# mit-han-lab/qserve

Hardware: AMD Instinct MI355X
Metric: decode tokens/sec/GPU Llama-3-8B W4A8KV4 bs=64 (higher is better)
Workload: dtype int8xint4->int32 (MFMA) + fp16; 1 GPU; Llama-3-8B W4A8 per-channel KV4 decode step, bs=64, context 1024->+512 (BASELINE.json configs[1]); global_batch=64, context_start=1030, parallelism=tp1, hipgraph=True, layers=32, launches_per_layer=8

## Files before the change

qserve_amd/csrc/attention.hip:

```cpp
#include "common.h"
#include "kv_quant.h"

namespace {

constexpr int TPB = 256;
constexpr int PAGE_TOK = 64;
constexpr int DH = 128;

__device__ __forceinline__ void nib8_to_h2(u32 x, h2 (&o)[4]) {
    const u32 t = x >> 8;
    u32 w0 = (x & 0x000F000Fu) | 0x64006400u;
    u32 w1 = (x & 0x00F000F0u) | 0x64006400u;
    u32 w2 = (t & 0x000F000Fu) | 0x64006400u;
    u32 w3 = (t & 0x00F000F0u) | 0x64006400u;
    const h2 k1024 = {(_Float16)1024.f, (_Float16)1024.f};
    const h2 k16 = {(_Float16)0.0625f, (_Float16)0.0625f};
    const h2 km64 = {(_Float16)-64.f, (_Float16)-64.f};
    o[0] = __builtin_bit_cast(h2, w0) - k1024;
    o[1] = __builtin_elementwise_fma(__builtin_bit_cast(h2, w1), k16, km64);
    o[2] = __builtin_bit_cast(h2, w2) - k1024;
    o[3] = __builtin_elementwise_fma(__builtin_bit_cast(h2, w3), k16, km64);
}

template <bool INT4>
// ... 546 lines not shown
        case 2: QS_LAUNCH_G(2); break;
        case 3: QS_LAUNCH_G(3); break;
        case 4: QS_LAUNCH_G(4); break;
        case 5: QS_LAUNCH_G(5); break;
        case 6: QS_LAUNCH_G(6); break;
        case 7: QS_LAUNCH_G(7); break;
        case 8: QS_LAUNCH_G(8); break;
        default:
            qs_set_error("single_query_attention: num_heads/num_kv_heads = %d not in 1..8", G);
            return QS_ENOSUP;
    }
#undef QS_LAUNCH_G
    return qs_launch_status("single_query_attention");
}

}

const float2* qs_rope_table(float base, int max_pos, hipStream_t st, int* len_out);
int qs_launch_decode_mfma(int G, dim3 grid, hipStream_t st, const _Float16* q, const _Float16* k, const _Float16* v,
                          const int64_t* kvp, const int* len, _Float16* out, int H, int Hkv, int64_t qs, int64_t kvs,
                          int mb, int timestep, float base, int max_pos, int nsplit, int kflags, int exp_flags,
                          const QsAttnQuant* quant, bool* fused);
int qs_launch_decode_mfma8(int G, dim3 grid, hipStream_t st, const _Float16* q, const _Float16* k, const _Float16* v,
                           const int64_t* kvp, const int* len, _Float16* out, int H, int Hkv, int64_t qs, int64_t kvs,
                           int mb, int timestep, float base, int max_pos, int nsplit);
namespace {

qs_flag g_attn_variant = 0;

int qs_attn_choose_splits(int blocks, int pages, int kv8, int fused_quant) {
    if (blocks >= 512 || pages < 4) return 1;
    const long F = kv8 ? 5000 : 4000, t_cu = kv8 ? 450 : 340, t_hbm_ps = kv8 ? 2540 : 1330;
    long best = -1;
    int best_n = 1;
    for (int n = 1; n <= 8; ++n) {
        if (n > 1 && pages / n < 2) break;
        const long rounds = ((long)blocks * n + 255) / 256;
        const long per_cu = rounds * pages * t_cu / n, chip = (long)blocks * pages * t_hbm_ps / 1000;
        const long cost = rounds * F + (per_cu > chip ? per_cu : chip) + (n > 1 ? 2500 + 300 * n + (fused_quant ? 3500 : 0) : 0);
        if (best < 0 || cost < best) best = cost, best_n = n;
    }
    return best_n;
}
struct AttnPlan {
    int family, nsplit, waves, kflags, exp_flags;
};
AttnPlan plan_attention(int batch, int H, int Hkv, int max_blocks, int timestep, bool int4, bool fused_quant, int variant) {
    const int G = H / Hkv;
    if (G < 1 || G > 8) {
        qs_set_error("single_query_attention: num_heads/num_kv_heads = %d not in 1..8", G);
        return {0};
    }
    if (variant == 1 || max_blocks > 192) return {3, 1, TPB / 64};
    int force_split = variant >= 100 ? variant - 100 : 0, exp_flags = 0;
    if (int4 && force_split >= 100) {
        exp_flags = force_split - 100;
        force_split = 0;
    }
    const int blocks = Hkv * batch;
    const int pages_max = (timestep + PAGE_TOK - 1) / PAGE_TOK;
    const int nsplit = force_split > 0 ? force_split : qs_attn_choose_splits(blocks, pages_max, int4 ? 0 : 1, int4 && fused_quant && H * DH <= 4096);
    if (int4) return {1, nsplit, QS_ATTN_WAVES_KV4, variant == 5 ? 2 : variant == 7 ? 1024 : 0, exp_flags};
    return {2, nsplit, QS_ATTN_WAVES_KV8};
}

int single_query_attention(const void* q, const void* k, const void* v, const int64_t* kv_pointers,
                           const int32_t* length_per_sample, void* out, int batch, int num_heads, int num_kv_heads,
                           int head_dim, int64_t q_stride0, int64_t kv_stride0, int max_blocks, int memory_max_seqlen,
                           int tokens_per_block, int size_per_token, int timestep, int rotary_embedding_dim,
                           float rotary_base, int neox_rotary_style, int int4_kv_cache, int kv_cache_with_zeros,
                           qs_stream_t stream, const QsAttnQuant* quant, bool* fused) {
    QS_REQUIRE(q && k && v && kv_pointers && out, "single_query_attention: null pointer");
    QS_REQUIRE(batch >= 0 && num_heads > 0 && num_kv_heads > 0 && num_heads % num_kv_heads == 0,
               "single_query_attention: bad head counts H=%d Hkv=%d", num_heads, num_kv_heads);
    (void)neox_rotary_style;
    if (head_dim != 128 || rotary_embedding_dim != 128 || tokens_per_block != 64 || !kv_cache_with_zeros) {
        qs_set_error("single_query_attention: only head_dim=128, rotary_dim=128, tokens_per_block=64 and "
                     "zero-point KV caches are supported (the variants the reference instantiates)");
        return QS_ENOSUP;
    }
    const int dhb = int4_kv_cache ? 64 : 128;
    QS_REQUIRE(size_per_token == num_kv_heads * dhb, "single_query_attention: size_per_token=%d, expected %d",
               size_per_token, num_kv_heads * dhb);
    QS_REQUIRE(max_blocks > 0 && memory_max_seqlen > 0, "single_query_attention: bad max_blocks / memory_max_seqlen");
    QS_REQUIRE(q_stride0 % 8 == 0 && kv_stride0 % 8 == 0 && q_stride0 >= (int64_t)num_heads * 128 && kv_stride0 >= (int64_t)num_kv_heads * 128,
               "single_query_attention: token strides must hold the token's heads and keep 16-byte alignment");
    QS_REQUIRE(((reinterpret_cast<uintptr_t>(q) | reinterpret_cast<uintptr_t>(k) | reinterpret_cast<uintptr_t>(v) |
                 reinterpret_cast<uintptr_t>(out)) & 15) == 0,
               "single_query_attention: q, k, v and out must be 16-byte aligned");
    if (batch == 0) return QS_OK;
    const AttnPlan plan = plan_attention(batch, num_heads, num_kv_heads, max_blocks, timestep, int4_kv_cache, quant != nullptr,
                                         g_attn_variant);
    if (!plan.family) return QS_ENOSUP;
    dim3 grid(num_kv_heads, batch);
    const int G = num_heads / num_kv_heads;
    hipStream_t st = (hipStream_t)stream;
    const _Float16 *q16 = (const _Float16*)q, *k16 = (const _Float16*)k, *v16 = (const _Float16*)v;
    if (plan.family == 1)
        return qs_launch_decode_mfma(G, grid, st, q16, k16, v16, kv_pointers, length_per_sample, (_Float16*)out, num_heads,
                                     num_kv_heads, q_stride0, kv_stride0, max_blocks, timestep, rotary_base, memory_max_seqlen,
                                     plan.nsplit, plan.kflags, plan.exp_flags, quant, fused);
    if (plan.family == 2)
        return qs_launch_decode_mfma8(G, grid, st, q16, k16, v16, kv_pointers, length_per_sample, (_Float16*)out, num_heads,
                                      num_kv_heads, q_stride0, kv_stride0, max_blocks, timestep, rotary_base, memory_max_seqlen,
                                      plan.nsplit);
    if (int4_kv_cache)
        return launch_decode<true>(G, grid, st, q16, k16, v16, kv_pointers, length_per_sample, (_Float16*)out, num_heads,
                                   num_kv_heads, q_stride0, kv_stride0, max_blocks, timestep, rotary_base);
    return launch_decode<false>(G, grid, st, q16, k16, v16, kv_pointers, length_per_sample, (_Float16*)out, num_heads,
                                num_kv_heads, q_stride0, kv_stride0, max_blocks, timestep, rotary_base);
}

}

extern "C" void qs_set_attention_variant(int variant) { g_attn_variant = variant; }
// ... 157 lines not shown
```

qserve_amd/csrc/attention_mfma.hip:

```cpp
#include "common.h"
#include "kv_quant.h"
#include <mutex>

namespace {

constexpr int PAGE_TOK = 64;
constexpr int DH = 128;
constexpr int DHB = 64;
constexpr int UT = 32;
constexpr int USB = UT * DHB;
constexpr int NW = QS_ATTN_WAVES_KV4;
constexpr int NWT = NW;
constexpr int QS_ATTNQ_CAP = 4096;
constexpr int QS_ATTNQ_ROW = 4096;
constexpr int SVC = NW - 1;
#ifndef QS_SEQ
#define QS_SEQ(x) asm volatile("" : "+v"(x))
#endif
constexpr int MAXP = 192;

typedef __attribute__((address_space(1))) uint8_t* g_u8;
typedef __attribute__((address_space(1))) uint16_t* g_u16;
__device__ __forceinline__ void wave_quant_store4(_Float16 v0, _Float16 v1, uint8_t* dst_, __half* scale_p_,
                                                  __half* zero_p_, int lane) {
    g_u8 dst = (g_u8)dst_;
    g_u16 scale_p = (g_u16)reinterpret_cast<uint16_t*>(scale_p_), zero_p = (g_u16)reinterpret_cast<uint16_t*>(zero_p_);
    const float mx = wave_max_dpp(fmaxf((float)v0, (float)v1));
    const float mn = wave_min_dpp(fminf((float)v0, (float)v1));
    const QParams p = make_qparams<true>(mn, mx);
    const unsigned u0 = quant_u8(v0, p), u1 = quant_u8(v1, p);
    dst[lane] = (uint8_t)((u0 & 0xFu) | (u1 << 4));
    if (lane == 0) {
        *scale_p = __builtin_bit_cast(uint16_t, p.scale);
        *zero_p = __builtin_bit_cast(uint16_t, p.zero);
    }
}

__device__ __forceinline__ u32 and_or(u32 x, u32 m, u32 c) {
    return (x & m) | c;
}

typedef __attribute__((address_space(3))) const uint8_t* lds_u8;

template <int G, int EXP = 0>
__global__ __launch_bounds__(NWT * 64, 4) void decode_attention_mfma_kernel(
    const _Float16* __restrict__ q, const _Float16* __restrict__ k, const _Float16* __restrict__ v,
    const int64_t* __restrict__ kv_pointers, const int* __restrict__ lengths, _Float16* __restrict__ out,
    int num_heads, int num_kv_heads, int64_t q_stride0, int64_t kv_stride0, int max_blocks, int timestep,
    float rope_base, const float2* __restrict__ rope_tab, int rope_tab_len, int nsplit, float* __restrict__ ws,
    int8_t* __restrict__ qout, __half* __restrict__ qscale, __half* __restrict__ qrowsum, unsigned* __restrict__ qcounters,
    int kflags) {
    __shared__ __attribute__((aligned(16))) uint8_t s_kv[2 * NW * 2 * USB];
    __shared__ __attribute__((aligned(16))) _Float16 s_meta[NW][2][4][UT];
    __shared__ __attribute__((aligned(16))) _Float16 s_q[G][DH];
    __shared__ __attribute__((aligned(16))) _Float16 s_qp[16][DH];
    __shared__ __attribute__((aligned(16))) _Float16 s_knew[DH];
    __shared__ __attribute__((aligned(16))) _Float16 s_vnew[DH];
    __shared__ float s_cur[16];
    __shared__ float2 s_qc[16];
    __shared__ float s_m[NW][G], s_l[NW][G];
    __shared__ int s_flag;

    const int tid = threadIdx.x, lane = tid & 63;
    const int wave = __builtin_amdgcn_readfirstlane(tid >> 6);
    const int hkv = blockIdx.x, b = blockIdx.y;
    __shared__ unsigned long long s_stamps[(EXP & 32) ? NWT * 16 : 1];
    auto stamp = [&](int i) {
        if constexpr (EXP & 32) {
            const unsigned long long t = __builtin_amdgcn_s_memtime();
            if (lane == 0) s_stamps[wave * 16 + i] = t;
        }
    };
    if constexpr (EXP & 32) {
        if (lane < 16) s_stamps[wave * 16 + lane] = 0;
    }
    stamp(0);
    if (!(kflags & 2)) {
        const u32 fa = (u32)(uintptr_t)(__attribute__((address_space(3))) void*)(&s_flag);
        if (tid == SVC * 64) asm volatile("ds_write_b32 %0, %1" ::"v"(fa), "v"(0));
        asm volatile("s_waitcnt lgkmcnt(0)\n\ts_barrier");
    }
    const _Float16* qb = q + (size_t)b * q_stride0 + (size_t)hkv * G * DH;
    const _Float16* kb = k + (size_t)b * kv_stride0 + (size_t)hkv * DH;
    const _Float16* vb = v + (size_t)b * kv_stride0 + (size_t)hkv * DH;
    auto uni_ptr = [](const void* x) -> uint64_t {
        return ((uint64_t)(u32)__builtin_amdgcn_readfirstlane((u32)((uint64_t)(uintptr_t)x >> 32)) << 32) |
               (uint64_t)(u32)__builtin_amdgcn_readfirstlane((u32)(uint64_t)(uintptr_t)x);
    };
    const uint64_t qb_s = uni_ptr(qb), kb_s = uni_ptr(kb), vb_s = uni_ptr(vb);
    const int64_t* ktab = kv_pointers + (size_t)b * 2 * max_blocks;
    const int64_t* vtab = ktab + max_blocks;
    const bool spec = (nsplit == 1 || blockIdx.z == 0);
    if (wave == SVC) {
        asm volatile("s_setprio 3");
        if constexpr (!(EXP & 4)) {
            const u32 lane4 = (u32)lane * 4u;
            auto glds4 = [&](uint64_t sb, const _Float16* dst) {
                const u32 ld = __builtin_amdgcn_readfirstlane((u32)(uintptr_t)(__attribute__((address_space(3))) const void*)dst);
                asm volatile("s_mov_b32 m0, %2\n\ts_nop 4\n\tglobal_load_lds_dword %0, %1" ::"v"(lane4), "s"(sb), "s"(ld) : "memory");
            };
#pragma unroll
            for (int h = 0; h < G; ++h) glds4(qb_s + (uint64_t)(h * DH * 2), &s_q[h][0]);
            glds4(kb_s, &s_knew[0]);
            glds4(vb_s, &s_vnew[0]);
        }
        stamp(5);
    }
    int64_t kpage0, vpage0, kpage7, vpage7;
    int len_raw, gen_raw;
    {
        const int p0 = (wave >> 1) < max_blocks ? (wave >> 1) : 0, p7 = ((wave + NW - 1) >> 1) < max_blocks ? ((wave + NW - 1) >> 1) : 0;
        const uint64_t a0 = uni_ptr(ktab + p0), a1 = uni_ptr(vtab + p0), a2 = uni_ptr(ktab + p7), a3 = uni_ptr(vtab + p7);
        const uint64_t a4 = uni_ptr(lengths ? (const void*)(lengths + b) : (const void*)ktab);
        const uint64_t a5 = uni_ptr(qcounters ? (const void*)(qcounters + b) : (const void*)ktab);
        asm volatile("s_load_dwordx2 %0, %6, 0x0\n\ts_load_dwordx2 %1, %7, 0x0\n\ts_load_dwordx2 %2, %8, 0x0\n\t"
                     "s_load_dwordx2 %3, %9, 0x0\n\ts_load_dword %4, %10, 0x0\n\ts_load_dword %5, %11, 0x0\n\ts_waitcnt lgkmcnt(0)"
                     : "=&s"(kpage0), "=&s"(vpage0), "=&s"(kpage7), "=&s"(vpage7), "=&s"(len_raw), "=&s"(gen_raw)
                     : "s"(a0), "s"(a1), "s"(a2), "s"(a3), "s"(a4), "s"(a5)
                     : "memory");
    }
    const int tl = lengths ? len_raw - 1 : timestep;
    if (tl < 0) return;
    stamp(1);
    const float inv_sqrt = 0.08838834764831845f;
    const float qk_scale = inv_sqrt * 1.4426950408889634f;
    constexpr int GP = G <= 4 ? 4 : 8;
    const int li = lane & 15, tg = lane >> 4;
// ... 338 lines not shown
            for (int j = 0; j < NS; ++j) {
                const float pe = __builtin_amdgcn_exp2f(sc[j] - m_new);
                l_part += pe;
                float ps = (float)(_Float16)(pe * vsf[j]);
                float pz = ps * vzf[j];
                if (!full && tok0 + j >= valid) {
                    ps = 0.f;
                    pz = 0.f;
                }
                corr += pz;
                psum += ps;
                pp[j] = ps;
            }
            if constexpr (GP == 4) {
                const int pk = (int)pack_h2(pp[0], pp[1]);
                pbv[0] = (u32)pk;
                pbv[1] = (u32)__builtin_amdgcn_update_dpp(0, pk, 0x104, 0xF, 0xF, true);
                pbv[2] = (u32)__builtin_amdgcn_update_dpp(0, pk, 0x108, 0xF, 0xF, true);
                pbv[3] = (u32)__builtin_amdgcn_update_dpp(0, pk, 0x10C, 0xF, 0xF, true);
            } else {
                const int pk0 = (int)pack_h2(pp[0], pp[1]), pk1 = (int)pack_h2(pp[2], pp[3]);
                pbv[0] = (u32)pk0;
                pbv[1] = (u32)pk1;
                pbv[2] = (u32)__builtin_amdgcn_update_dpp(0, pk0, 0x108, 0xF, 0xF, true);
                pbv[3] = (u32)__builtin_amdgcn_update_dpp(0, pk1, 0x108, 0xF, 0xF, true);
            }
        }
        {
            const h8 pB = __builtin_bit_cast(h8, (v4u){pbv[0], pbv[1], pbv[2], pbv[3]});
            u32 raw[8];
#pragma unroll
            for (int jj = 0; jj < 8; ++jj) {
                raw[jj] = *(const __attribute__((address_space(3))) u32*)(vl + (16 * (jj >> 2) + (jj & 3)) * DHB);
            }
#pragma unroll
            for (int bb = 0; bb < 4; ++bb) {
                u32 lo[4], hi[4];
#pragma unroll
                for (int pq = 0; pq < 4; ++pq) {
                    const u32 W = __builtin_amdgcn_perm(raw[2 * pq + 1], raw[2 * pq], 0x0c000c00u | bb | ((4u + bb) << 16));
                    lo[pq] = and_or(W, c_lo, c_magic);
                    hi[pq] = and_or(W, c_hi, c_magic);
                }
                const h8 a_lo = __builtin_bit_cast(h8, (v4u){lo[0], lo[1], lo[2], lo[3]});
                const h8 a_hi = __builtin_bit_cast(h8, (v4u){hi[0], hi[1], hi[2], hi[3]});
                acc[2 * bb] = __builtin_amdgcn_mfma_f32_16x16x32_f16(a_lo, pB, acc[2 * bb], 0, 0, 0);
                acc[2 * bb + 1] = __builtin_amdgcn_mfma_f32_16x16x32_f16(a_hi, pB, acc[2 * bb + 1], 0, 0, 0);
            }
        }
        asm volatile("s_waitcnt lgkmcnt(0) ; QS_LOOP_END" ::: "memory");
        if (it < 2) stamp(6 + 2 * it);
        if (has2) dma_b(vpage_next, u2 & 1, slot, valid2);
    }

    const u32 lid2 = fresh_lane_id();
    const int li2 = lid2 & 15, tg2 = lid2 >> 4, tid2 = wave * 64 + (int)lid2;
    if constexpr (GP == 4) {
        l_part += xor_lane(l_part, lid2, 4);
        corr += xor_lane(corr, lid2, 4);
        psum += xor_lane(psum, lid2, 4);
    }
    l_part += xor_lane(l_part, lid2, 8);
    corr += xor_lane(corr, lid2, 8);
    psum += xor_lane(psum, lid2, 8);
    l_part += xor_lane(l_part, lid2, 16);
    l_part += xor_lane(l_part, lid2, 32);
    corr += xor_lane(corr, lid2, 16);
    corr += xor_lane(corr, lid2, 32);
    psum += xor_lane(psum, lid2, 16);
    psum += xor_lane(psum, lid2, 32);
    if constexpr (!(EXP & 4)) {
        if (wave == SVC && !svc_free) new_token_work();
    }
    asm volatile("s_waitcnt vmcnt(0)" ::: "memory");
    stamp(12);
    __syncthreads();
    stamp(13);
    constexpr int OS = DH + 4;
    float (*s_o)[G][OS] = reinterpret_cast<float (*)[G][OS]>(&s_kv[0]);
    static_assert(sizeof(float) * NW * G * OS <= sizeof(s_kv), "merge area must fit the page buffers");
    if (li2 < G) {
#pragma unroll
        for (int e = 0; e < 8; ++e)
#pragma unroll
            for (int r = 0; r < 4; ++r)
                s_o[wave][li2][8 * (4 * tg2 + r) + e] = ((e & 1) ? acc[e][r] * 0.0625f : acc[e][r]) - (corr + ((e & 1) ? 64.f : 1024.f) * psum);
        if (tg2 == 0) {
            s_m[wave][li2] = m_run;
            s_l[wave][li2] = l_part;
        }
    }
    __syncthreads();
    stamp(14);
    for (int o = tid2; o < G * DH; o += NWT * 64) {
        const int h = o / DH, d = o % DH;
        float M = z == 0 ? s_cur[h] : -3.0e38f;
#pragma unroll
        for (int w = 0; w < NW; ++w) M = fmaxf(M, s_m[w][h]);
        const float pc = z == 0 ? __builtin_amdgcn_exp2f(s_cur[h] - M) : 0.f;
        float num = pc * (float)((EXP & 4) ? vb[d] : s_vnew[d]), den = pc;
#pragma unroll
        for (int w = 0; w < NW; ++w) {
            const float f = __builtin_amdgcn_exp2f(s_m[w][h] - M);
            num += f * s_o[w][h][d];
            den += f * s_l[w][h];
        }
        if (nsplit == 1) {
            const _Float16 res = (_Float16)(num / (den + 1.e-6f));
            if (qout) reinterpret_cast<_Float16*>(&s_meta[0][0][0])[o] = res;
            else out[((size_t)b * num_heads + (size_t)hkv * G + h) * DH + d] = res;
        } else {
            float* pw = ws + ((((size_t)b * num_kv_heads + hkv) * nsplit + z) * G + h) * (DH + 2);
            pw[d] = num;
            if (d == 0) {
                pw[DH] = M * 0.6931471805599453f;
                pw[DH + 1] = den;
            }
        }
    }
    if (nsplit == 1 && qout) {
        __syncthreads();
        const int hidden = num_heads * DH;
        const unsigned tag = (unsigned)gen_raw + 1u;
        if (tid2 < G * 16) {
            const v4u x = reinterpret_cast<const v4u*>(&s_meta[0][0][0])[tid2];
            *reinterpret_cast<v4u*>(out + ((size_t)b * num_heads + (size_t)hkv * G) * DH + tid2 * 8) = x;
        }
        v2u* const xrow = reinterpret_cast<v2u*>(qcounters + QS_ATTNQ_CAP) + (size_t)b * (QS_ATTNQ_ROW / 2);
        const int own_lo = (num_kv_heads - 1) * G * DH;
        if ((G == 4 || G == 8) && !(kflags & 1024)) {
            float* const sm = reinterpret_cast<float*>(&s_kv[0]);
            v4u* const gran = reinterpret_cast<v4u*>(xrow);
            if (wave == 0) {
                const int ln = (int)lid2;
                float amax = 0.f, s0 = 0.f, s1 = 0.f;
                {
                    const h8 vv = __builtin_bit_cast(h8, reinterpret_cast<const v4u*>(&s_meta[0][0][0])[ln]);
#pragma unroll
                    for (int j = 0; j < 8; ++j) {
                        const float f = (float)vv[j];
                        s0 += f;
                        QS_SEQ(s0);
                        amax = fmaxf(amax, fabsf(f));
                    }
                }
                if (G == 8) {
                    const h8 vv = __builtin_bit_cast(h8, reinterpret_cast<const v4u*>(&s_meta[0][0][0])[64 + ln]);
#pragma unroll
                    for (int j = 0; j < 8; ++j) {
                        const float f = (float)vv[j];
                        s1 += f;
                        QS_SEQ(s1);
                        amax = fmaxf(amax, fabsf(f));
                    }
                }
                amax = wave_max(amax);
                s0 = wave_sum(s0);
                if (G == 8) s1 = wave_sum(s1);
                v4u mine = {__builtin_bit_cast(u32, amax), __builtin_bit_cast(u32, s0), __builtin_bit_cast(u32, s1), tag};
                if (ln == 0 && !((kflags & 64) && b == 0 && hkv == 0) && !(kflags & 512)) {
                    v4u* const dst = gran + hkv;
                    asm volatile("global_store_dwordx4 %0, %1, off sc0 sc1" ::"v"(dst), "v"(mine) : "memory");
                }
                const __amdgpu_buffer_rsrc_t grs = __builtin_amdgcn_make_buffer_rsrc(gran, 0, num_kv_heads * 16, 0x00020000);
                const bool peer = ln < num_kv_heads && ln != hkv;
                const u32 goff = ln < num_kv_heads ? (u32)ln * 16u : 0xFFFFFF00u;
                const int spin_cap = (kflags & 256) ? 1 : (kflags & 64) ? 4096 : QS_SPIN_CAP;
                int polls = 0;
                v4u g;
                for (;;) {
                    g = __builtin_amdgcn_raw_buffer_load_b128(grs, goff, 0, 17);
                    if (!__builtin_amdgcn_ballot_w64(peer && g.w != tag)) break;
                    if (++polls >= spin_cap) {
                        if (ln == 0 && !(kflags & 256))
                            atomicOr(qcounters + QS_ATTNQ_CAP + (size_t)QS_ATTNQ_CAP * QS_ATTNQ_ROW, QS_ERR_ATTN_HANDOVER);
                        break;
                    }
                    __builtin_amdgcn_s_sleep(1);
                }
                if (ln == hkv) g = mine;
                const u32 gx = g.x, gy = g.y, gz = g.z;
                float am = ln < num_kv_heads ? __builtin_bit_cast(float, gx) : 0.f;
                am = wave_max(am);
                float bs;
                if (G == 4) {
                    bs = ln < num_kv_heads ? __builtin_bit_cast(float, gy) : -0.0f;
                } else {
                    const int src = (ln >> 1) < num_kv_heads ? (ln >> 1) : 0;
                    const int yv = __builtin_amdgcn_ds_bpermute(4 * src, (int)gy), zv = __builtin_amdgcn_ds_bpermute(4 * src, (int)gz);
                    bs = (ln >> 1) < num_kv_heads ? __builtin_bit_cast(float, (ln & 1) ? zv : yv) : -0.0f;
                }
                const float tot = wave_sum(bs);
                if (ln == 0) {
                    sm[0] = am;
                    sm[1] = tot;
                }
            }
            __syncthreads();
            const float r = sm[0];
            if (tid2 < G * 16) {
                const h8 vv = __builtin_bit_cast(h8, reinterpret_cast<const v4u*>(&s_meta[0][0][0])[tid2]);
                float f[8];
#pragma unroll
                for (int j = 0; j < 8; ++j) f[j] = (float)vv[j];
                qs_store_q8(qout + (size_t)b * hidden + (size_t)hkv * G * DH + tid2 * 8, f, 127.0f / r);
            }
            if (hkv == num_kv_heads - 1 && tid2 == 0) {
                qscale[b] = __float2half_rn(r / 127.0f);
                if (qrowsum) qrowsum[b] = __float2half_rn(sm[1]);
                qcounters[b] = tag;
            }
        } else if (hkv != num_kv_heads - 1) {
            for (int e = tid2; e < G * DH / 2 && !((kflags & 64) && b == 0 && hkv == 0) && !(kflags & 512); e += NWT * 64) {
                v2u gr;
                gr.x = reinterpret_cast<const u32*>(&s_meta[0][0][0])[e];
                gr.y = tag;
                v2u* const dst = xrow + (size_t)hkv * (G * DH / 2) + e;
                asm volatile("global_store_dwordx2 %0, %1, off sc0 sc1" ::"v"(dst), "v"(gr) : "memory");
            }
        } else {
            const __amdgpu_buffer_rsrc_t xrs = __builtin_amdgcn_make_buffer_rsrc(xrow, 0, QS_ATTNQ_ROW * 4, 0x00020000);
            v4u raw[2] = {{0, 0, 0, 0}, {0, 0, 0, 0}};
            if (tid2 < 256) {
                const int i0 = tid2 * 8, i1 = (256 + tid2) * 8;
                const bool p0 = i0 < own_lo, p1 = i1 < own_lo;
                const u32 o0 = p0 ? (u32)i0 * 4u : 0xFFFFFF00u, o1 = p1 ? (u32)i1 * 4u : 0xFFFFFF00u;
                const int spin_cap = (kflags & 256) ? 1 : (kflags & 64) ? 4096 : QS_SPIN_CAP;
                int polls = 0;
                for (;;) {
                    const v4u g00 = __builtin_amdgcn_raw_buffer_load_b128(xrs, o0, 0, 17);
                    const v4u g01 = __builtin_amdgcn_raw_buffer_load_b128(xrs, o0, 16, 17);
                    const v4u g10 = __builtin_amdgcn_raw_buffer_load_b128(xrs, o1, 0, 17);
                    const v4u g11 = __builtin_amdgcn_raw_buffer_load_b128(xrs, o1, 16, 17);
                    const int m0 = (g00.y != tag) | (g00.w != tag) | (g01.y != tag) | (g01.w != tag);
                    const int m1 = (g10.y != tag) | (g10.w != tag) | (g11.y != tag) | (g11.w != tag);
                    raw[0] = (v4u){g00.x, g00.z, g01.x, g01.z};
                    raw[1] = (v4u){g10.x, g10.z, g11.x, g11.z};
                    if (!__builtin_amdgcn_ballot_w64((p0 && m0) || (p1 && m1))) break;
                    if (++polls >= spin_cap) {
                        if ((tid2 & 63) == 0 && !(kflags & 256))
                            atomicOr(qcounters + QS_ATTNQ_CAP + (size_t)QS_ATTNQ_CAP * QS_ATTNQ_ROW, QS_ERR_ATTN_HANDOVER);
                        break;
                    }
                    __builtin_amdgcn_s_sleep(1);
                }
                if (!p0 && i0 < hidden) raw[0] = reinterpret_cast<const v4u*>(&s_meta[0][0][0])[(i0 - own_lo) >> 3];
                if (!p1 && i1 < hidden) raw[1] = reinterpret_cast<const v4u*>(&s_meta[0][0][0])[(i1 - own_lo) >> 3];
            }
            float* const sm = reinterpret_cast<float*>(&s_kv[0]);
            float amax = 0.f, sum[2] = {0.f, 0.f};
            if (tid2 < 256) {
#pragma unroll
                for (int c = 0; c < 2; ++c) {
                    const int i = (c * 256 + tid2) * 8;
                    if (i < hidden) {
                        const h8 vv = __builtin_bit_cast(h8, raw[c]);
#pragma unroll
                        for (int j = 0; j < 8; ++j) {
                            const float f = (float)vv[j];
                            sum[c] += f;
                            QS_SEQ(sum[c]);
                            amax = fmaxf(amax, fabsf(f));
                        }
                    }
                }
                amax = wave_max(amax);
                if (qrowsum) {
                    sum[0] = wave_sum(sum[0]);
                    sum[1] = wave_sum(sum[1]);
                }
                if ((tid2 & 63) == 0) {
                    sm[tid2 >> 6] = amax;
                    sm[4 + (tid2 >> 6)] = sum[0];
                    sm[8 + (tid2 >> 6)] = sum[1];
                }
            }
            __syncthreads();
            if (tid2 < 256) {
                float r = sm[0];
#pragma unroll
                for (int w = 1; w < 4; ++w) r = fmaxf(r, sm[w]);
                float s2 = 0.f;
                if (qrowsum && tid2 < 64) s2 = wave_sum(tid2 < (hidden + 511) / 512 ? sm[4 + tid2] : -0.0f);
                if (tid2 == 0) {
                    qscale[b] = __float2half_rn(r / 127.0f);
                    if (qrowsum) qrowsum[b] = __float2half_rn(s2);
                    qcounters[b] = tag;
                }
                const float mul = 127.0f / r;
#pragma unroll
                for (int c = 0; c < 2; ++c) {
                    const int i = (c * 256 + tid2) * 8;
                    if (i < hidden) {
                        const h8 vv = __builtin_bit_cast(h8, raw[c]);
                        float f[8];
#pragma unroll
                        for (int j = 0; j < 8; ++j) f[j] = (float)vv[j];
                        qs_store_q8(qout + (size_t)b * hidden + i, f, mul);
                    }
                }
            }
        }
    }
    stamp(15);
    if constexpr (EXP & 32) {
        if (lane < 16)
            reinterpret_cast<unsigned long long*>(ws)[(((size_t)b * gridDim.x + hkv) * NWT + wave) * 16 + lane] = s_stamps[wave * 16 + lane];
    }
}

__global__ __launch_bounds__(DH) void decode_attention_merge_kernel(const float* __restrict__ ws, _Float16* __restrict__ out,
                                                                    int num_heads, int num_kv_heads, int G, int nsplit) {
    const int b = blockIdx.y, hq = blockIdx.x, d = threadIdx.x;
    const int hkv = hq / G, h = hq % G;
    const float* base = ws + (((size_t)b * num_kv_heads + hkv) * nsplit * G + h) * (DH + 2);
    const size_t zs = (size_t)G * (DH + 2);
    float M = -3.0e38f;
    for (int zz = 0; zz < nsplit; ++zz) M = fmaxf(M, base[zz * zs + DH]);
    float num = 0.f, den = 0.f;
    for (int zz = 0; zz < nsplit; ++zz) {
        const float f = __expf(base[zz * zs + DH] - M);
        num += f * base[zz * zs + d];
        den += f * base[zz * zs + DH + 1];
    }
    out[((size_t)b * num_heads + hq) * DH + d] = (_Float16)(num / (den + 1.e-6f));
}

__global__ void rope_table_kernel(float2* __restrict__ tab, int max_pos, float base) {
    const int i = blockIdx.x * blockDim.x + threadIdx.x;
    if (i >= max_pos * 64) return;
    const RopeCS cs = rope_coef(i & 63, i >> 6, base, DH);
    tab[i] = make_float2(cs.c, cs.s);
}

struct RopeTable {
    float2* tab = nullptr;
    int len = 0;
    float base = 0.f;
};
constexpr int ROPE_SLOTS = 8;
RopeTable g_rope[16][ROPE_SLOTS];

}

const float2* qs_rope_table(float base, int max_pos, hipStream_t st, int* len_out) {
    static std::mutex g_rope_mutex;
    std::lock_guard<std::mutex> lock(g_rope_mutex);
    int dev = 0;
    *len_out = 0;
    if (hipGetDevice(&dev) != hipSuccess || dev < 0 || dev >= 16) return nullptr;
    if (max_pos > 32768) max_pos = 32768;
    if (max_pos <= 0) return nullptr;
    RopeTable* slot = nullptr;
    for (int i = 0; i < ROPE_SLOTS; ++i) {
        RopeTable& r = g_rope[dev][i];
        if (r.tab && r.base == base && r.len >= max_pos) {
            *len_out = r.len;
            return r.tab;
        }
        if (!r.tab && !slot) slot = &r;
// ... 97 lines not shown
int qs_attn_reset_handoff() {
    int dev = 0;
    if (hipGetDevice(&dev) != hipSuccess || dev < 0 || dev >= 16) return QS_OK;
    const size_t bytes = (size_t)QS_ATTNQ_CAP * 4 + (size_t)QS_ATTNQ_CAP * QS_ATTNQ_ROW * 4 + 64;
    for (int slot = 0; slot < QS_MAX_STREAM_SLOTS; ++slot) {
        if (!g_qcounters[dev][slot]) continue;
        hipError_t e = hipMemset(g_qcounters[dev][slot], 0, bytes);
        if (e == hipSuccess) e = hipDeviceSynchronize();
        if (e != hipSuccess) {
            qs_set_error("qs_device_reset (attention): %s", hipGetErrorString(e));
            return (int)e;
        }
    }
    return QS_OK;
}

int qs_launch_decode_mfma(int G, dim3 grid, hipStream_t st, const _Float16* q, const _Float16* k, const _Float16* v,
                          const int64_t* kvp, const int* len, _Float16* out, int H, int Hkv, int64_t qs, int64_t kvs,
                          int mb, int timestep, float base, int max_pos, int nsplit, int kflags, int exp_flags,
                          const QsAttnQuant* quant, bool* fused) {
    int tab_len = 0;
    const float2* tab = qs_rope_table(base, max_pos, st, &tab_len);
    const int blocks = (int)(grid.x * grid.y);
    float* ws = nullptr;
    if (nsplit > 1) {
        const size_t per_split = (size_t)blocks * G * (DH + 2) * sizeof(float);
        if (per_split * nsplit > qs_split_workspace_capacity()) nsplit = (int)(qs_split_workspace_capacity() / per_split);
        ws = nsplit > 1 ? qs_split_workspace(per_split * nsplit, st) : nullptr;
        if (!ws) nsplit = 1;
    }
    grid.z = nsplit;
    int8_t* qout = nullptr;
    __half *qscale = nullptr, *qsum = nullptr;
    unsigned* qcnt = nullptr;
    const bool sum_order_ok = !(quant && qs_get_row_sum_order() && quant->qsum);
    if (quant && sum_order_ok && nsplit == 1 && H * DH <= 4096 && (qcnt = qs_attn_quant_counters(st, (int)grid.y))) {
        qout = quant->qout;
        qscale = reinterpret_cast<__half*>(quant->qscale);
        qsum = reinterpret_cast<__half*>(quant->qsum);
        *fused = true;
        if (g_inject_fault & 2) kflags |= 64, g_inject_fault &= ~2;
    }
#define QS_LAUNCH_G(GG)                                                                                             \
    hipLaunchKernelGGL((decode_attention_mfma_kernel<GG>), grid, dim3(NWT * 64), 0, st, q, k, v, kvp, len, out, H, Hkv, \
                       qs, kvs, mb, timestep, base, tab, tab_len, nsplit, ws, qout, qscale, qsum, qcnt, kflags)
#define QS_LAUNCH_EXP(E)                                                                                              \
    case E:                                                                                                            \
        hipLaunchKernelGGL((decode_attention_mfma_kernel<4, E>), grid, dim3(NWT * 64), 0, st, q, k, v, kvp, len, out, H,  \
                           Hkv, qs, kvs, mb, timestep, base, tab, tab_len, nsplit, ws, qout, qscale, qsum, qcnt, kflags); \
        return qs_launch_status("single_query_attention")
#ifdef QS_TIMING
    if (const char* e = getenv("QS_ATTN_KFLAGS")) kflags = atoi(e);
    if (exp_flags & 32) {
        ws = qs_split_workspace((size_t)blocks * NWT * 16 * 8, st);
        if (!ws) exp_flags = 0;
    }
    if (G == 4 && exp_flags > 0 && nsplit == 1) {
        switch (exp_flags) {
            QS_LAUNCH_EXP(1);
            QS_LAUNCH_EXP(2);
            QS_LAUNCH_EXP(4);
            QS_LAUNCH_EXP(6);
            QS_LAUNCH_EXP(32);
            default: break;
        }
    }
#endif
    switch (G) {
        case 1: QS_LAUNCH_G(1); break;
        case 2: QS_LAUNCH_G(2); break;
        case 3: QS_LAUNCH_G(3); break;
        case 4: QS_LAUNCH_G(4); break;
        case 5: QS_LAUNCH_G(5); break;
        case 6: QS_LAUNCH_G(6); break;
        case 7: QS_LAUNCH_G(7); break;
        case 8: QS_LAUNCH_G(8); break;
        default:
            qs_set_error("single_query_attention: num_heads/num_kv_heads = %d not in 1..8", G);
            return QS_ENOSUP;
    }
#undef QS_LAUNCH_G
    if (nsplit > 1)
        hipLaunchKernelGGL(decode_attention_merge_kernel, dim3(H, grid.y), dim3(DH), 0, st, ws, out, H, Hkv, G, nsplit);
    return qs_launch_status("single_query_attention");
}
```

Measured before the change: 22920 tokens/s.

## Drop pre-merge barrier and let wave 0 merge partials in the fused-quant tail

Restructures the attention epilogue. Each wave now writes its partial outputs into its own ring slot of the page buffer, so the barrier before that write is removed. In the fused quantize path with G=4/8, wave 0 alone merges the per-wave partials, publishes amax/rowsum, and writes fp16 and int8 outputs directly, skipping the staging through shared memory and a second barrier. A kflag keeps the old tail for comparison. The gain is fewer block-wide syncs and shorter serial tail latency, at the cost of doing all merge work in a single wave and more code complexity.

```diff
diff --git a/qserve_amd/csrc/attention.hip b/qserve_amd/csrc/attention.hip
--- a/qserve_amd/csrc/attention.hip
+++ b/qserve_amd/csrc/attention.hip
@@ -622,6 +622,8 @@
         return {0};
     }
     if (variant == 1 || max_blocks > 192) return {3, 1, TPB / 64};
+    const bool old_tail = variant == 8 || (variant >= 1000 && variant < 1100);
+    if (variant >= 1000 && variant < 1100) variant = variant > 1000 ? variant - 900 : 0;
     int force_split = variant >= 100 ? variant - 100 : 0, exp_flags = 0;
     if (int4 && force_split >= 100) {
         exp_flags = force_split - 100;
@@ -630,7 +632,7 @@
     const int blocks = Hkv * batch;
     const int pages_max = (timestep + PAGE_TOK - 1) / PAGE_TOK;
     const int nsplit = force_split > 0 ? force_split : qs_attn_choose_splits(blocks, pages_max, int4 ? 0 : 1, int4 && fused_quant && H * DH <= 4096);
-    if (int4) return {1, nsplit, QS_ATTN_WAVES_KV4, variant == 5 ? 2 : variant == 7 ? 1024 : 0, exp_flags};
+    if (int4) return {1, nsplit, QS_ATTN_WAVES_KV4, variant == 5 ? 2 : variant == 7 ? 1024 : old_tail ? 2048 : 0, exp_flags};
     return {2, nsplit, QS_ATTN_WAVES_KV8};
 }
 
diff --git a/qserve_amd/csrc/attention_mfma.hip b/qserve_amd/csrc/attention_mfma.hip
--- a/qserve_amd/csrc/attention_mfma.hip
+++ b/qserve_amd/csrc/attention_mfma.hip
@@ -1,6 +1,7 @@
 #include "common.h"
 #include "kv_quant.h"
 #include <mutex>
+#include <type_traits>
 
 namespace {
 
@@ -17,6 +18,7 @@
 #ifndef QS_SEQ
 #define QS_SEQ(x) asm volatile("" : "+v"(x))
 #endif
+constexpr int NST = 20;
 constexpr int MAXP = 192;
 
 typedef __attribute__((address_space(1))) uint8_t* g_u8;
@@ -64,15 +66,15 @@
     const int tid = threadIdx.x, lane = tid & 63;
     const int wave = __builtin_amdgcn_readfirstlane(tid >> 6);
     const int hkv = blockIdx.x, b = blockIdx.y;
-    __shared__ unsigned long long s_stamps[(EXP & 32) ? NWT * 16 : 1];
+    __shared__ unsigned long long s_stamps[(EXP & 32) ? NWT * NST : 1];
     auto stamp = [&](int i) {
         if constexpr (EXP & 32) {
             const unsigned long long t = __builtin_amdgcn_s_memtime();
-            if (lane == 0) s_stamps[wave * 16 + i] = t;
+            if (lane == 0) s_stamps[wave * NST + i] = t;
         }
     };
     if constexpr (EXP & 32) {
-        if (lane < 16) s_stamps[wave * 16 + lane] = 0;
+        if (lane < NST) s_stamps[wave * NST + lane] = 0;
     }
     stamp(0);
     if (!(kflags & 2)) {
@@ -517,6 +519,7 @@
         if (it < 2) stamp(6 + 2 * it);
         if (has2) dma_b(vpage_next, u2 & 1, slot, valid2);
     }
+    stamp(17);
 
     const u32 lid2 = fresh_lane_id();
     const int li2 = lid2 & 15, tg2 = lid2 >> 4, tid2 = wave * 64 + (int)lid2;
@@ -539,94 +542,90 @@
     }
     asm volatile("s_waitcnt vmcnt(0)" ::: "memory");
     stamp(12);
-    __syncthreads();
-    stamp(13);
     constexpr int OS = DH + 4;
-    float (*s_o)[G][OS] = reinterpret_cast<float (*)[G][OS]>(&s_kv[0]);
     static_assert(sizeof(float) * NW * G * OS <= sizeof(s_kv), "merge area must fit the page buffers");
-    if (li2 < G) {
-#pragma unroll
-        for (int e = 0; e < 8; ++e)
-#pragma unroll
-            for (int r = 0; r < 4; ++r)
-                s_o[wave][li2][8 * (4 * tg2 + r) + e] = ((e & 1) ? acc[e][r] * 0.0625f : acc[e][r]) - (corr + ((e & 1) ? 64.f : 1024.f) * psum);
-        if (tg2 == 0) {
-            s_m[wave][li2] = m_run;
-            s_l[wave][li2] = l_part;
-        }
-    }
-    __syncthreads();
-    stamp(14);
-    for (int o = tid2; o < G * DH; o += NWT * 64) {
-        const int h = o / DH, d = o % DH;
-        float M = z == 0 ? s_cur[h] : -3.0e38f;
-#pragma unroll
-        for (int w = 0; w < NW; ++w) M = fmaxf(M, s_m[w][h]);
-        const float pc = z == 0 ? __builtin_amdgcn_exp2f(s_cur[h] - M) : 0.f;
-        float num = pc * (float)((EXP & 4) ? vb[d] : s_vnew[d]), den = pc;
-#pragma unroll
-        for (int w = 0; w < NW; ++w) {
-            const float f = __builtin_amdgcn_exp2f(s_m[w][h] - M);
-            num += f * s_o[w][h][d];
-            den += f * s_l[w][h];
-        }
-        if (nsplit == 1) {
-            const _Float16 res = (_Float16)(num / (den + 1.e-6f));
-            if (qout) reinterpret_cast<_Float16*>(&s_meta[0][0][0])[o] = res;
-            else out[((size_t)b * num_heads + (size_t)hkv * G + h) * DH + d] = res;
-        } else {
-            float* pw = ws + ((((size_t)b * num_kv_heads + hkv) * nsplit + z) * G + h) * (DH + 2);
-            pw[d] = num;
-            if (d == 0) {
-                pw[DH] = M * 0.6931471805599453f;
-                pw[DH + 1] = den;
-            }
-        }
-    }
-    if (nsplit == 1 && qout) {
+    static_assert(sizeof(float) * 4 * OS <= 2 * USB, "four heads' partials must fit one wave's ring");
+    const bool allgather = (G == 4 || G == 8) && !(kflags & 1024);
+    auto tail = [&](auto nt) {
+        constexpr bool NT = decltype(nt)::value;
+        if constexpr (!NT) {
+            __syncthreads();
+            stamp(13);
+        }
+        auto prow = [&](int w, int h) -> float* {
+            if constexpr (NT) return reinterpret_cast<float*>(&s_kv[((h >> 2) * NW + w) * (2 * USB)]) + (h & 3) * OS;
+            else return reinterpret_cast<float*>(&s_kv[0]) + (w * G + h) * OS;
+        };
+        if (li2 < G) {
+            float* const po = prow(wave, li2);
+#pragma unroll
+            for (int e = 0; e < 8; ++e)
+#pragma unroll
+                for (int r = 0; r < 4; ++r)
+                    po[8 * (4 * tg2 + r) + e] = ((e & 1) ? acc[e][r] * 0.0625f : acc[e][r]) - (corr + ((e & 1) ? 64.f : 1024.f) * psum);
+            if (tg2 == 0) {
+                s_m[wave][li2] = m_run;
+                s_l[wave][li2] = l_part;
+            }
+        }
         __syncthreads();
+        stamp(14);
         const int hidden = num_heads * DH;
         const unsigned tag = (unsigned)gen_raw + 1u;
-        if (tid2 < G * 16) {
-            const v4u x = reinterpret_cast<const v4u*>(&s_meta[0][0][0])[tid2];
-            *reinterpret_cast<v4u*>(out + ((size_t)b * num_heads + (size_t)hkv * G) * DH + tid2 * 8) = x;
-        }
         v2u* const xrow = reinterpret_cast<v2u*>(qcounters + QS_ATTNQ_CAP) + (size_t)b * (QS_ATTNQ_ROW / 2);
-        const int own_lo = (num_kv_heads - 1) * G * DH;
-        if ((G == 4 || G == 8) && !(kflags & 1024)) {
-            float* const sm = reinterpret_cast<float*>(&s_kv[0]);
-            v4u* const gran = reinterpret_cast<v4u*>(xrow);
+        if (NT && nsplit == 1 && qout && allgather) {
             if (wave == 0) {
-                const int ln = (int)lid2;
-                float amax = 0.f, s0 = 0.f, s1 = 0.f;
-                {
-                    const h8 vv = __builtin_bit_cast(h8, reinterpret_cast<const v4u*>(&s_meta[0][0][0])[ln]);
+                const int ln = (int)lid2, d0 = 8 * (ln & 15);
+                constexpr int NC = G >= 4 ? G / 4 : 1;
+                h8 vv[NC];
+#pragma unroll
+                for (int c = 0; c < NC; ++c) {
+                    const int h = 4 * c + (ln >> 4);
+                    float M = s_cur[h];
+#pragma unroll
+                    for (int w = 0; w < NW; ++w) M = fmaxf(M, s_m[w][h]);
+                    const float pc = __builtin_amdgcn_exp2f(s_cur[h] - M);
+                    float num[8], den = pc;
+#pragma unroll
+                    for (int j = 0; j < 8; ++j) num[j] = pc * (float)((EXP & 4) ? vb[d0 + j] : s_vnew[d0 + j]);
+#pragma unroll
+                    for (int w = 0; w < NW; ++w) {
+                        const float f = __builtin_amdgcn_exp2f(s_m[w][h] - M);
+                        const float* const pr = prow(w, h) + d0;
+                        const v4f a0 = *reinterpret_cast<const v4f*>(pr), a1 = *reinterpret_cast<const v4f*>(pr + 4);
+#pragma unroll
+                        for (int j = 0; j < 4; ++j) {
+                            num[j] += f * a0[j];
+                            num[4 + j] += f * a1[j];
+                        }
+                        den += f * s_l[w][h];
+                    }
+#pragma unroll
+                    for (int j = 0; j < 8; ++j) vv[c][j] = (_Float16)(num[j] / (den + 1.e-6f));
+                }
+                stamp(9);
+                float amax = 0.f, ssum[NC];
+#pragma unroll
+                for (int c = 0; c < NC; ++c) {
+                    ssum[c] = 0.f;
 #pragma unroll
                     for (int j = 0; j < 8; ++j) {
-                        const float f = (float)vv[j];
-                        s0 += f;
-                        QS_SEQ(s0);
+                        const float f = (float)vv[c][j];
+                        ssum[c] += f;
+                        QS_SEQ(ssum[c]);
                         amax = fmaxf(amax, fabsf(f));
                     }
                 }
-                if (G == 8) {
-                    const h8 vv = __builtin_bit_cast(h8, reinterpret_cast<const v4u*>(&s_meta[0][0][0])[64 + ln]);
-#pragma unroll
-                    for (int j = 0; j < 8; ++j) {
-                        const float f = (float)vv[j];
-                        s1 += f;
-                        QS_SEQ(s1);
-                        amax = fmaxf(amax, fabsf(f));
-                    }
-                }
                 amax = wave_max(amax);
-                s0 = wave_sum(s0);
-                if (G == 8) s1 = wave_sum(s1);
+                const float s0 = wave_sum(ssum[0]);
+                const float s1 = NC > 1 ? wave_sum(ssum[NC - 1]) : 0.f;
+                v4u* const gran = reinterpret_cast<v4u*>(xrow);
                 v4u mine = {__builtin_bit_cast(u32, amax), __builtin_bit_cast(u32, s0), __builtin_bit_cast(u32, s1), tag};
                 if (ln == 0 && !((kflags & 64) && b == 0 && hkv == 0) && !(kflags & 512)) {
                     v4u* const dst = gran + hkv;
                     asm volatile("global_store_dwordx4 %0, %1, off sc0 sc1" ::"v"(dst), "v"(mine) : "memory");
                 }
+                stamp(10);
                 const __amdgpu_buffer_rsrc_t grs = __builtin_amdgcn_make_buffer_rsrc(gran, 0, num_kv_heads * 16, 0x00020000);
                 const bool peer = ln < num_kv_heads && ln != hkv;
                 const u32 goff = ln < num_kv_heads ? (u32)ln * 16u : 0xFFFFFF00u;
@@ -643,6 +642,7 @@
                     }
                     __builtin_amdgcn_s_sleep(1);
                 }
+                stamp(16);
                 if (ln == hkv) g = mine;
                 const u32 gx = g.x, gy = g.y, gz = g.z;
                 float am = ln < num_kv_heads ? __builtin_bit_cast(float, gx) : 0.f;
@@ -656,121 +656,255 @@
                     bs = (ln >> 1) < num_kv_heads ? __builtin_bit_cast(float, (ln & 1) ? zv : yv) : -0.0f;
                 }
                 const float tot = wave_sum(bs);
-                if (ln == 0) {
-                    sm[0] = am;
-                    sm[1] = tot;
-                }
-            }
+#pragma unroll
+                for (int c = 0; c < NC; ++c) {
+                    const size_t col = (size_t)hkv * G * DH + c * 512 + ln * 8;
+                    *reinterpret_cast<v4u*>(out + (size_t)b * num_heads * DH + col) = __builtin_bit_cast(v4u, vv[c]);
+                    float f[8];
+#pragma unroll
+                    for (int j = 0; j < 8; ++j) f[j] = (float)vv[c][j];
+                    qs_store_q8(qout + (size_t)b * hidden + col, f, 127.0f / am);
+                }
+                if (hkv == num_kv_heads - 1 && ln == 0) {
+                    qscale[b] = __float2half_rn(am / 127.0f);
+                    if (qrowsum) qrowsum[b] = __float2half_rn(tot);
+                    qcounters[b] = tag;
+                }
+            }
+            return;
+        }
+        const bool direct = NT && nsplit == 1 && qout && hkv != num_kv_heads - 1;
+        for (int o = tid2; o < G * DH; o += NWT * 64) {
+            const int h = o / DH, d = o % DH;
+            float M = z == 0 ? s_cur[h] : -3.0e38f;
+#pragma unroll
+            for (int w = 0; w < NW; ++w) M = fmaxf(M, s_m[w][h]);
+            const float pc = z == 0 ? __builtin_amdgcn_exp2f(s_cur[h] - M) : 0.f;
+            float num = pc * (float)((EXP & 4) ? vb[d] : s_vnew[d]), den = pc;
+#pragma unroll
+            for (int w = 0; w < NW; ++w) {
+                const float f = __builtin_amdgcn_exp2f(s_m[w][h] - M);
+                num += f * prow(w, h)[d];
+                den += f * s_l[w][h];
+            }
+            if (nsplit == 1) {
+                const _Float16 res = (_Float16)(num / (den + 1.e-6f));
+                if (qout) reinterpret_cast<_Float16*>(&s_meta[0][0][0])[o] = res;
+                else out[((size_t)b * num_heads + (size_t)hkv * G + h) * DH + d] = res;
+                if (direct) {
+                    const int mine = (int)__builtin_bit_cast(uint16_t, res);
+                    const int nb = __builtin_amdgcn_update_dpp(0, mine, 0xB1, 0xF, 0xF, true);
+                    if (!(o & 1) && !((kflags & 64) && b == 0 && hkv == 0) && !(kflags & 512)) {
+                        v2u gr;
+                        gr.x = (u32)mine | ((u32)nb << 16);
+                        gr.y = tag;
+                        v2u* const dst = xrow + (size_t)hkv * (G * DH / 2) + (o >> 1);
+                        asm volatile("global_store_dwordx2 %0, %1, off sc0 sc1" ::"v"(dst), "v"(gr) : "memory");
+                    }
+                    stamp(10);
+                }
+            } else {
+                float* pw = ws + ((((size_t)b * num_kv_heads + hkv) * nsplit + z) * G + h) * (DH + 2);
+                pw[d] = num;
+                if (d == 0) {
+                    pw[DH] = M * 0.6931471805599453f;
+                    pw[DH + 1] = den;
+                }
+            }
+        }
+        stamp(9);
+        if (nsplit == 1 && qout) {
             __syncthreads();
-            const float r = sm[0];
             if (tid2 < G * 16) {
-                const h8 vv = __builtin_bit_cast(h8, reinterpret_cast<const v4u*>(&s_meta[0][0][0])[tid2]);
-                float f[8];
-#pragma unroll
-                for (int j = 0; j < 8; ++j) f[j] = (float)vv[j];
-                qs_store_q8(qout + (size_t)b * hidden + (size_t)hkv * G * DH + tid2 * 8, f, 127.0f / r);
-            }
-            if (hkv == num_kv_heads - 1 && tid2 == 0) {
-                qscale[b] = __float2half_rn(r / 127.0f);
-                if (qrowsum) qrowsum[b] = __float2half_rn(sm[1]);
-                qcounters[b] = tag;
-            }
-        } else if (hkv != num_kv_heads - 1) {
-            for (int e = tid2; e < G * DH / 2 && !((kflags & 64) && b == 0 && hkv == 0) && !(kflags & 512); e += NWT * 64) {
-                v2u gr;
-                gr.x = reinterpret_cast<const u32*>(&s_meta[0][0][0])[e];
-                gr.y = tag;
-                v2u* const dst = xrow + (size_t)hkv * (G * DH / 2) + e;
-                asm volatile("global_store_dwordx2 %0, %1, off sc0 sc1" ::"v"(dst), "v"(gr) : "memory");
-            }
-        } else {
-            const __amdgpu_buffer_rsrc_t xrs = __builtin_amdgcn_make_buffer_rsrc(xrow, 0, QS_ATTNQ_ROW * 4, 0x00020000);
-            v4u raw[2] = {{0, 0, 0, 0}, {0, 0, 0, 0}};
-            if (tid2 < 256) {
-                const int i0 = tid2 * 8, i1 = (256 + tid2) * 8;
-                const bool p0 = i0 < own_lo, p1 = i1 < own_lo;
-                const u32 o0 = p0 ? (u32)i0 * 4u : 0xFFFFFF00u, o1 = p1 ? (u32)i1 * 4u : 0xFFFFFF00u;
-                const int spin_cap = (kflags & 256) ? 1 : (kflags & 64) ? 4096 : QS_SPIN_CAP;
-                int polls = 0;
-                for (;;) {
-                    const v4u g00 = __builtin_amdgcn_raw_buffer_load_b128(xrs, o0, 0, 17);
-                    const v4u g01 = __builtin_amdgcn_raw_buffer_load_b128(xrs, o0, 16, 17);
-                    const v4u g10 = __builtin_amdgcn_raw_buffer_load_b128(xrs, o1, 0, 17);
-                    const v4u g11 = __builtin_amdgcn_raw_buffer_load_b128(xrs, o1, 16, 17);
-                    const int m0 = (g00.y != tag) | (g00.w != tag) | (g01.y != tag) | (g01.w != tag);
-                    const int m1 = (g10.y != tag) | (g10.w != tag) | (g11.y != tag) | (g11.w != tag);
-                    raw[0] = (v4u){g00.x, g00.z, g01.x, g01.z};
-                    raw[1] = (v4u){g10.x, g10.z, g11.x, g11.z};
-                    if (!__builtin_amdgcn_ballot_w64((p0 && m0) || (p1 && m1))) break;
-                    if (++polls >= spin_cap) {
-                        if ((tid2 & 63) == 0 && !(kflags & 256))
-                            atomicOr(qcounters + QS_ATTNQ_CAP + (size_t)QS_ATTNQ_CAP * QS_ATTNQ_ROW, QS_ERR_ATTN_HANDOVER);
-                        break;
-                    }
-                    __builtin_amdgcn_s_sleep(1);
-                }
-                if (!p0 && i0 < hidden) raw[0] = reinterpret_cast<const v4u*>(&s_meta[0][0][0])[(i0 - own_lo) >> 3];
-                if (!p1 && i1 < hidden) raw[1] = reinterpret_cast<const v4u*>(&s_meta[0][0][0])[(i1 - own_lo) >> 3];
-            }
-            float* const sm = reinterpret_cast<float*>(&s_kv[0]);
-            float amax = 0.f, sum[2] = {0.f, 0.f};
-            if (tid2 < 256) {
-#pragma unroll
-                for (int c = 0; c < 2; ++c) {
-                    const int i = (c * 256 + tid2) * 8;
-                    if (i < hidden) {
-                        const h8 vv = __builtin_bit_cast(h8, raw[c]);
-#pragma unroll
+                const v4u x = reinterpret_cast<const v4u*>(&s_meta[0][0][0])[tid2];
+                *reinterpret_cast<v4u*>(out + ((size_t)b * num_heads + (size_t)hkv * G) * DH + tid2 * 8) = x;
+            }
+            const int own_lo = (num_kv_heads - 1) * G * DH;
+            if (allgather) {
+                float* const sm = reinterpret_cast<float*>(&s_kv[0]);
+                v4u* const gran = reinterpret_cast<v4u*>(xrow);
+                if (wave == 0) {
+                    const int ln = (int)lid2;
+                    float amax = 0.f, s0 = 0.f, s1 = 0.f;
+                    {
+                        const h8 vv = __builtin_bit_cast(h8, reinterpret_cast<const v4u*>(&s_meta[0][0][0])[ln]);
+    #pragma unroll
                         for (int j = 0; j < 8; ++j) {
                             const float f = (float)vv[j];
-                            sum[c] += f;
-                            QS_SEQ(sum[c]);
+                            s0 += f;
+                            QS_SEQ(s0);
                             amax = fmaxf(amax, fabsf(f));
                         }
                     }
-                }
-                amax = wave_max(amax);
-                if (qrowsum) {
-                    sum[0] = wave_sum(sum[0]);
-                    sum[1] = wave_sum(sum[1]);
-                }
-                if ((tid2 & 63) == 0) {
-                    sm[tid2 >> 6] = amax;
-                    sm[4 + (tid2 >> 6)] = sum[0];
-                    sm[8 + (tid2 >> 6)] = sum[1];
-                }
-            }
-            __syncthreads();
-            if (tid2 < 256) {
-                float r = sm[0];
-#pragma unroll
-                for (int w = 1; w < 4; ++w) r = fmaxf(r, sm[w]);
-                float s2 = 0.f;
-                if (qrowsum && tid2 < 64) s2 = wave_sum(tid2 < (hidden + 511) / 512 ? sm[4 + tid2] : -0.0f);
-                if (tid2 == 0) {
+                    if (G == 8) {
+                        const h8 vv = __builtin_bit_cast(h8, reinterpret_cast<const v4u*>(&s_meta[0][0][0])[64 + ln]);
+    #pragma unroll
+                        for (int j = 0; j < 8; ++j) {
+                            const float f = (float)vv[j];
+                            s1 += f;
+                            QS_SEQ(s1);
+                            amax = fmaxf(amax, fabsf(f));
+                        }
+                    }
+                    amax = wave_max(amax);
+                    s0 = wave_sum(s0);
+                    if (G == 8) s1 = wave_sum(s1);
+                    v4u mine = {__builtin_bit_cast(u32, amax), __builtin_bit_cast(u32, s0), __builtin_bit_cast(u32, s1), tag};
+                    if (ln == 0 && !((kflags & 64) && b == 0 && hkv == 0) && !(kflags & 512)) {
+                        v4u* const dst = gran + hkv;
+                        asm volatile("global_store_dwordx4 %0, %1, off sc0 sc1" ::"v"(dst), "v"(mine) : "memory");
+                    }
+                    stamp(10);
+                    const __amdgpu_buffer_rsrc_t grs = __builtin_amdgcn_make_buffer_rsrc(gran, 0, num_kv_heads * 16, 0x00020000);
+                    const bool peer = ln < num_kv_heads && ln != hkv;
+                    const u32 goff = ln < num_kv_heads ? (u32)ln * 16u : 0xFFFFFF00u;
+                    const int spin_cap = (kflags & 256) ? 1 : (kflags & 64) ? 4096 : QS_SPIN_CAP;
+                    int polls = 0;
+                    v4u g;
+                    for (;;) {
+                        g = __builtin_amdgcn_raw_buffer_load_b128(grs, goff, 0, 17);
+                        if (!__builtin_amdgcn_ballot_w64(peer && g.w != tag)) break;
+                        if (++polls >= spin_cap) {
+                            if (ln == 0 && !(kflags & 256))
+                                atomicOr(qcounters + QS_ATTNQ_CAP + (size_t)QS_ATTNQ_CAP * QS_ATTNQ_ROW, QS_ERR_ATTN_HANDOVER);
+                            break;
+                        }
+                        __builtin_amdgcn_s_sleep(1);
+                    }
+                    stamp(16);
+                    if (ln == hkv) g = mine;
+                    const u32 gx = g.x, gy = g.y, gz = g.z;
+                    float am = ln < num_kv_heads ? __builtin_bit_cast(float, gx) : 0.f;
+                    am = wave_max(am);
+                    float bs;
+                    if (G == 4) {
+                        bs = ln < num_kv_heads ? __builtin_bit_cast(float, gy) : -0.0f;
+                    } else {
+                        const int src = (ln >> 1) < num_kv_heads ? (ln >> 1) : 0;
+                        const int yv = __builtin_amdgcn_ds_bpermute(4 * src, (int)gy), zv = __builtin_amdgcn_ds_bpermute(4 * src, (int)gz);
+                        bs = (ln >> 1) < num_kv_heads ? __builtin_bit_cast(float, (ln & 1) ? zv : yv) : -0.0f;
+                    }
+                    const float tot = wave_sum(bs);
+                    if (ln == 0) {
+                        sm[0] = am;
+                        sm[1] = tot;
+                    }
+                }
+                __syncthreads();
+                const float r = sm[0];
+                if (tid2 < G * 16) {
+                    const h8 vv = __builtin_bit_cast(h8, reinterpret_cast<const v4u*>(&s_meta[0][0][0])[tid2]);
+                    float f[8];
+    #pragma unroll
+                    for (int j = 0; j < 8; ++j) f[j] = (float)vv[j];
+                    qs_store_q8(qout + (size_t)b * hidden + (size_t)hkv * G * DH + tid2 * 8, f, 127.0f / r);
+                }
+                if (hkv == num_kv_heads - 1 && tid2 == 0) {
                     qscale[b] = __float2half_rn(r / 127.0f);
-                    if (qrowsum) qrowsum[b] = __float2half_rn(s2);
+                    if (qrowsum) qrowsum[b] = __float2half_rn(sm[1]);
                     qcounters[b] = tag;
                 }
-                const float mul = 127.0f / r;
-#pragma unroll
-                for (int c = 0; c < 2; ++c) {
-                    const int i = (c * 256 + tid2) * 8;
-                    if (i < hidden) {
-                        const h8 vv = __builtin_bit_cast(h8, raw[c]);
-                        float f[8];
-#pragma unroll
-                        for (int j = 0; j < 8; ++j) f[j] = (float)vv[j];
-                        qs_store_q8(qout + (size_t)b * hidden + i, f, mul);
-                    }
-                }
-            }
-        }
-    }
+            } else if (hkv != num_kv_heads - 1) {
+                for (int e = tid2; !NT && e < G * DH / 2 && !((kflags & 64) && b == 0 && hkv == 0) && !(kflags & 512); e += NWT * 64) {
+                    v2u gr;
+                    gr.x = reinterpret_cast<const u32*>(&s_meta[0][0][0])[e];
+                    gr.y = tag;
+                    v2u* const dst = xrow + (size_t)hkv * (G * DH / 2) + e;
+                    asm volatile("global_store_dwordx2 %0, %1, off sc0 sc1" ::"v"(dst), "v"(gr) : "memory");
+                }
+                if constexpr (!NT) stamp(10);
+            } else {
+                const __amdgpu_buffer_rsrc_t xrs = __builtin_amdgcn_make_buffer_rsrc(xrow, 0, QS_ATTNQ_ROW * 4, 0x00020000);
+                v4u raw[2] = {{0, 0, 0, 0}, {0, 0, 0, 0}};
+                if (tid2 < 256) {
+                    const int i0 = tid2 * 8, i1 = (256 + tid2) * 8;
+                    const bool p0 = i0 < own_lo, p1 = i1 < own_lo;
+                    const u32 o0 = p0 ? (u32)i0 * 4u : 0xFFFFFF00u, o1 = p1 ? (u32)i1 * 4u : 0xFFFFFF00u;
+                    const int spin_cap = (kflags & 256) ? 1 : (kflags & 64) ? 4096 : QS_SPIN_CAP;
+                    int polls = 0;
+                    for (;;) {
+                        const v4u g00 = __builtin_amdgcn_raw_buffer_load_b128(xrs, o0, 0, 17);
+                        const v4u g01 = __builtin_amdgcn_raw_buffer_load_b128(xrs, o0, 16, 17);
+                        const v4u g10 = __builtin_amdgcn_raw_buffer_load_b128(xrs, o1, 0, 17);
+                        const v4u g11 = __builtin_amdgcn_raw_buffer_load_b128(xrs, o1, 16, 17);
+                        const int m0 = (g00.y != tag) | (g00.w != tag) | (g01.y != tag) | (g01.w != tag);
+                        const int m1 = (g10.y != tag) | (g10.w != tag) | (g11.y != tag) | (g11.w != tag);
+                        raw[0] = (v4u){g00.x, g00.z, g01.x, g01.z};
+                        raw[1] = (v4u){g10.x, g10.z, g11.x, g11.z};
+                        if (!__builtin_amdgcn_ballot_w64((p0 && m0) || (p1 && m1))) break;
+                        if (++polls >= spin_cap) {
+                            if ((tid2 & 63) == 0 && !(kflags & 256))
+                                atomicOr(qcounters + QS_ATTNQ_CAP + (size_t)QS_ATTNQ_CAP * QS_ATTNQ_ROW, QS_ERR_ATTN_HANDOVER);
+                            break;
+                        }
+                        __builtin_amdgcn_s_sleep(1);
+                    }
+                    stamp(16);
+                    if (!p0 && i0 < hidden) raw[0] = reinterpret_cast<const v4u*>(&s_meta[0][0][0])[(i0 - own_lo) >> 3];
+                    if (!p1 && i1 < hidden) raw[1] = reinterpret_cast<const v4u*>(&s_meta[0][0][0])[(i1 - own_lo) >> 3];
+                }
+                float* const sm = reinterpret_cast<float*>(&s_kv[0]);
+                float amax = 0.f, sum[2] = {0.f, 0.f};
+                if (tid2 < 256) {
+    #pragma unroll
+                    for (int c = 0; c < 2; ++c) {
+                        const int i = (c * 256 + tid2) * 8;
+                        if (i < hidden) {
+                            const h8 vv = __builtin_bit_cast(h8, raw[c]);
+    #pragma unroll
+                            for (int j = 0; j < 8; ++j) {
+                                const float f = (float)vv[j];
+                                sum[c] += f;
+                                QS_SEQ(sum[c]);
+                                amax = fmaxf(amax, fabsf(f));
+                            }
+                        }
+                    }
+                    amax = wave_max(amax);
+                    if (qrowsum) {
+                        sum[0] = wave_sum(sum[0]);
+                        sum[1] = wave_sum(sum[1]);
+                    }
+                    if ((tid2 & 63) == 0) {
+                        sm[tid2 >> 6] = amax;
+                        sm[4 + (tid2 >> 6)] = sum[0];
+                        sm[8 + (tid2 >> 6)] = sum[1];
+                    }
+                }
+                __syncthreads();
+                if (tid2 < 256) {
+                    float r = sm[0];
+    #pragma unroll
+                    for (int w = 1; w < 4; ++w) r = fmaxf(r, sm[w]);
+                    float s2 = 0.f;
+                    if (qrowsum && tid2 < 64) s2 = wave_sum(tid2 < (hidden + 511) / 512 ? sm[4 + tid2] : -0.0f);
+                    if (tid2 == 0) {
+                        qscale[b] = __float2half_rn(r / 127.0f);
+                        if (qrowsum) qrowsum[b] = __float2half_rn(s2);
+                        qcounters[b] = tag;
+                    }
+                    const float mul = 127.0f / r;
+    #pragma unroll
+                    for (int c = 0; c < 2; ++c) {
+                        const int i = (c * 256 + tid2) * 8;
+                        if (i < hidden) {
+                            const h8 vv = __builtin_bit_cast(h8, raw[c]);
+                            float f[8];
+    #pragma unroll
+                            for (int j = 0; j < 8; ++j) f[j] = (float)vv[j];
+                            qs_store_q8(qout + (size_t)b * hidden + i, f, mul);
+                        }
+                    }
+                }
+            }
+        }
+    };
+    if (kflags & 2048) tail(std::false_type{});
+    else tail(std::true_type{});
     stamp(15);
     if constexpr (EXP & 32) {
-        if (lane < 16)
-            reinterpret_cast<unsigned long long*>(ws)[(((size_t)b * gridDim.x + hkv) * NWT + wave) * 16 + lane] = s_stamps[wave * 16 + lane];
+        if (lane < NST)
+            reinterpret_cast<unsigned long long*>(ws)[(((size_t)b * gridDim.x + hkv) * NWT + wave) * NST + lane] = s_stamps[wave * NST + lane];
     }
 }
 
@@ -974,7 +1108,7 @@
 #ifdef QS_TIMING
     if (const char* e = getenv("QS_ATTN_KFLAGS")) kflags = atoi(e);
     if (exp_flags & 32) {
-        ws = qs_split_workspace((size_t)blocks * NWT * 16 * 8, st);
+        ws = qs_split_workspace((size_t)blocks * NWT * NST * 8, st);
         if (!ws) exp_flags = 0;
     }
     if (G == 4 && exp_flags > 0 && nsplit == 1) {
```

Result: no change. 22940 tokens/s (median of 4 runs) (+0.1%).
